# Bioconductor/SparseArray

Measured on AMD Instinct MI355X. Metric: GNZ/s, SVT crossprod(svt, dense) 1e6x1e4 @1% nnz, higher is better.
Workload: dtype f64

## Files before the change

include/svt_hip.h:

```cpp
#ifndef SVT_HIP_H
#define SVT_HIP_H

#include <stddef.h>
#include <stdint.h>

#ifdef __cplusplus
extern "C" {
#endif

#define SVT_UNSUPPORTED 1

#define SVT_LGLSXP 10
#define SVT_INTSXP 13
#define SVT_REALSXP 14

#define SVT_OP_ANYNA            1
#define SVT_OP_COUNTNAS         2
#define SVT_OP_ANY              3
#define SVT_OP_ALL              4
#define SVT_OP_MIN              5
#define SVT_OP_MAX              6
#define SVT_OP_RANGE            7
#define SVT_OP_SUM              8
#define SVT_OP_PROD             9
// ... 102 lines not shown
int svt_dev_crossprod_prepared(const svt_dev_csc *A, const void *ws, int K,
			       double *out, int64_t out_stride_c,
			       int64_t out_stride_k, void *stream);
int svt_dev_crossprod_csc_dense(const svt_dev_csc *A, const void *Y,
				int64_t ldY, int K, int tr_y, double *out,
				int64_t out_stride_c, int64_t out_stride_k,
				void *ws, size_t ws_bytes, void *stream);

typedef struct svt_dev_pbc svt_dev_pbc;
svt_dev_pbc *svt_dev_pbc_build(const svt_dev_csc *A, int CBW, int WPB, int logR);
void svt_dev_pbc_release(svt_dev_pbc *P);
void svt_dev_pbc_trim(void);
size_t svt_dev_pbc_bytes(const svt_dev_pbc *P);
size_t svt_dev_crossprod_pbc_ws_bytes(const svt_dev_pbc *P, int K);
int svt_dev_crossprod_pbc(const svt_dev_pbc *P, const svt_dev_csc *A,
			  const double *Y, int64_t ldY, int K, int tr_y,
			  double *out, int64_t out_stride_c,
			  int64_t out_stride_k, void *ws, size_t ws_bytes,
			  void *stream);

void svt_dev_pbc_set_spare_cus(int n);
int svt_dev_pbc_spare_cus(void);

void svt_dev_pbc_set_gather_pacing(int dsync, int spin);

void svt_dev_pbc_set_round_launches(int on);

int svt_dev_crossprod_pbc_from(const svt_dev_pbc *P, const svt_dev_csc *A,
			       const double *Y, int64_t ldY, int K, int tr_y,
			       double *out, int64_t out_stride_c,
			       int64_t out_stride_k, void *ws, size_t ws_bytes,
			       void *stream, int64_t first_col);

int svt_dev_crossprod_pbc_phase(const svt_dev_pbc *P, const svt_dev_csc *A,
				const double *Y, int64_t ldY, int K, int tr_y,
				double *out, int64_t out_stride_c,
				int64_t out_stride_k, void *ws, size_t ws_bytes,
				void *stream, int phase);

int svt_dev_colstats(const svt_dev_csc *A, int opcode, int na_rm,
		     double center, int64_t inner, void *out, int *warn_flag,
		     void *stream);

size_t svt_dev_colmedians_ws_bytes(int64_t nnz, int64_t ncol);
int svt_dev_colmedians(const svt_dev_csc *A, int na_rm, double *out, void *ws, size_t ws_bytes,
		       void *stream);
// ... 59 lines not shown
```

sparsearray_amd/_hip.py:

```python
from __future__ import annotations

import ctypes
import os

_HERE = os.path.dirname(os.path.abspath(__file__))
LIB_PATH = os.path.join(_HERE, "libsvt_hip_tuning.so" if os.environ.get("SVT_HIP_TUNING") == "1"
                        else "libsvt_hip.so")

EXPORTS = [
    "svt_init", "svt_last_error", "svt_device_arch", "svt_set_devices", "svt_get_devices", "svt_set_shard_min_nnz",
    "svt_crossprod2_SVT_mat", "svt_crossprod2_mat_SVT",
    "svt_crossprod2_SVT_SVT", "svt_crossprod1_SVT",
    "svt_matmul_SVT_mat", "svt_matmul_SVT_SVT", "svt_tcrossprod1_SVT", "svt_tcrossprod2_SVT_SVT",
    "svt_colMedians_SVT", "svt_rowMedians_SVT", "svt_dev_colmedians_ws_bytes", "svt_dev_colmedians",
    "svt_resident_set_limit", "svt_resident_clear", "svt_resident_stats", "svt_dev_pbc_bytes", "svt_dev_pbc_set_spare_cus", "svt_dev_pbc_spare_cus", "svt_dev_pbc_set_gather_pacing", "svt_dev_pbc_set_round_launches", "svt_dev_matmul_csc_csc_ws_bytes", "svt_dev_matmul_csc_csc", "svt_dev_rowsums_prepare", "svt_dev_rowsums_prepared", "svt_dev_rowsum_gid_bytes", "svt_dev_rowsum_prepare", "svt_dev_rowsum_prepared", "svt_dev_matmul_csc_csc_prepare", "svt_dev_matmul_csc_csc_prepared",
    "svt_dev_crossprod_csc_csc_ws_bytes", "svt_dev_crossprod_csc_csc", "svt_dev_crossprod_csc_csc_set_panel", "svt_sparse_crossprod_set_cost", "svt_dev_crossprod_csc_csc_dense_buffer",
    "svt_summarize_SVT", "svt_colStats_out_Rtype", "svt_colStats_SVT",
    "svt_rowStats_SVT", "svt_rowsum_SVT", "svt_colsum_SVT",
    "svt_rowsum_dgCMatrix", "svt_colsum_dgCMatrix",
    "svt_colMins_dgCMatrix", "svt_colMaxs_dgCMatrix", "svt_colRanges_dgCMatrix", "svt_colVars_dgCMatrix",
    "svt_upload", "svt_wrap_device_csc", "svt_release",
    "svt_dev_crossprod_ws_bytes", "svt_dev_crossprod_csc_dense",
    "svt_dev_dense_prepare", "svt_dev_crossprod_prepared",
    "svt_dev_pbc_build", "svt_dev_pbc_release", "svt_dev_pbc_trim",
    "svt_dev_crossprod_pbc_ws_bytes", "svt_dev_crossprod_pbc", "svt_dev_crossprod_pbc_phase", "svt_dev_crossprod_pbc_from",
    "svt_get_num_procs", "svt_get_max_threads", "svt_set_max_threads", "svt_dev_aperm_ws_bytes", "svt_dev_aperm_perm_ws_bytes", "svt_dev_aperm", "svt_dev_aperm_route_counts", "svt_aperm_SVT", "svt_transpose_2D_SVT", "svt_dev_transpose_ws_bytes", "svt_dev_transpose", "svt_dev_set_box_nnz", "svt_dev_boxed_calls", "svt_dev_colstats", "svt_dev_rowstats_ws_bytes", "svt_dev_rowsums", "svt_dev_rowsum",
]


class HipBackendError(RuntimeError):
    pass


_lib = None
_ready = False


def load_library() -> ctypes.CDLL:
# ... 59 lines not shown
```

sparsearray_amd/csrc/kernels_mult_pbc.hip:

```cpp
#include "svt_common.h"

#include <string.h>

#include <mutex>

#include "svt_scan.h"

typedef double d16 __attribute__((ext_vector_type(16)));
typedef double d8 __attribute__((ext_vector_type(8)));

struct svt_dev_pbc {
	int64_t nrow, ncol, nnz, nrec;
	int CBW, WPB, logR;
	int kind;
	int64_t ngroups, nblocks, npanels;
	uint4 *rec;
	int64_t *tile_ptr;
	int *col_has_na;
	int64_t max_leaf_nnz;
	mutable hipStream_t use_s[4];
	mutable int nuse;
	mutable bool use_overflow;
	int device;
};

#define PCH 256
__device__ inline int64_t pbc_stagger_batch(int stag_mode, int w, int64_t nb)
{
	const int g = w >> 2;
	switch (stag_mode) {
	case 0: return 0;
	case 1: return w & 1;
	case 2: return w & 3;
	case 3: return g & 1;
	case 4: return w & 7;
	case 5: return (w * nb) >> 4;
// ... 28 lines not shown
					  int64_t hi, int64_t key)
{
	while (lo < hi) {
		const int64_t mid = (lo + hi) >> 1;
		if ((int64_t) row[mid] < key) lo = mid + 1; else hi = mid;
	}
	return lo;
}

#define PBC_BATCH 4
#define PBC_SLACK 320
#define PBC_TP_PAD 8

__device__ inline void pbc1_store(uint4 *rec, int64_t ridx, uint32_t meta, double x)
{
	char *base = (char *) rec + (ridx >> 3) * 96;
	((uint32_t *) base)[ridx & 7] = meta;
	((double *) (base + 32))[ridx & 7] = x;
}

template <int MODE, int FMT>
__global__ void __launch_bounds__(64)
pbc_pass_kernel(const int64_t *__restrict__ col_ptr, const int32_t *__restrict__ row_idx,
		const double *__restrict__ val, int64_t ncol, int CBW, int logR,
		int64_t npanels, int64_t *__restrict__ counts_or_ptr,
		uint4 *__restrict__ rec, int *__restrict__ col_has_na, int stag_mode, int tile_flags)
{
	constexpr int BATCH = FMT == 1 ? 8 : PBC_BATCH;
	__shared__ int64_t fill[PCH];
	const int lane = threadIdx.x;
	const int64_t wv = blockIdx.x;
	const int64_t p0 = (int64_t) blockIdx.y * PCH;
	const int64_t p1 = p0 + PCH < npanels ? p0 + PCH : npanels;
#define TILE_OF(P) (wv * npanels + (P))
	for (int i = lane; i < PCH; i += 64)
		fill[i] = (MODE == 1 && p0 + i < npanels) ? counts_or_ptr[TILE_OF(p0 + i)] : 0;
	__syncthreads();
	const int64_t c0 = wv * CBW;
	const int64_t c1 = c0 + CBW < ncol ? c0 + CBW : ncol;
	for (int64_t c = c0; c < c1; c++) {
		const int64_t beg = col_ptr[c], end = col_ptr[c + 1];
		const int64_t lo = lower_bound_row(row_idx, beg, end, p0 << logR);
		const int64_t hi = lower_bound_row(row_idx, lo, end, p1 << logR);
		int saw_na = 0;
		for (int64_t k0 = lo; k0 < hi; k0 += 64) {
			const int64_t k = k0 + lane;
			const bool active = k < hi;
			const int32_t r = active ? row_idx[k] : 0;
			const int p = active ? (int) (((int64_t) r >> logR) - p0) : -1;
			const int prev_p = __shfl_up(p, 1, 64);
			const int next_p = __shfl_down(p, 1, 64);
			const bool is_first = active && (lane == 0 || p != prev_p);
			const bool is_last = active && (lane == 63 || p != next_p);
			const unsigned long long firsts = __ballot(is_first);
			const unsigned long long below = firsts & ((lane == 63) ? ~0ULL : ((2ULL << lane) - 1));
			const int seg_lane = 63 - __clzll(below | 1ULL);
			const int rank = lane - seg_lane;
			int64_t pos = 0;
			if (active) pos = fill[p] + rank;
			__syncthreads();
			if (MODE == 1 && active) {
				const double x = val[k];
// ... 37 lines not shown
				const int64_t nb = (stop - start) >> 3;
				int64_t bi = pbc_stagger_batch(stag_mode, w, nb);
				if (bi > nb - 1) bi = nb - 1;
				atomicOr((unsigned int *) ((char *) rec + ((start >> 3) + bi) * 96), 0x4000u);
			}
		}
	}
#undef TILE_OF
}

#define PBC_IMG_BYTES 24576
#define PBC_SC_KEEP 4

__device__ inline void pbc1_put(char *img, int64_t ridx, uint32_t meta, double x)
{
	char *b = img + (ridx >> 3) * 96;
	((uint32_t *) b)[ridx & 7] = meta;
	((double *) (b + 32))[ridx & 7] = x;
}

#define PBC_COUNT_MAXPANELS 36000
__global__ void __launch_bounds__(1024)
pbc_count_stream_kernel(const int64_t *__restrict__ col_ptr, const int32_t *__restrict__ row_idx, int64_t ncol,
			int CBW, int logR, int64_t npanels, int64_t *__restrict__ counts,
			int32_t *__restrict__ bounds, int64_t nchunks, int cshift)
{
	extern __shared__ uint32_t pbc_hist[];
	const int lane = threadIdx.x & 63, w = threadIdx.x >> 6;
	const int64_t g = blockIdx.x;
	for (int64_t p = threadIdx.x; p < npanels; p += 1024) pbc_hist[p] = 0;
	__syncthreads();
	const int64_t c0 = g * CBW, c1 = c0 + CBW < ncol ? c0 + CBW : ncol;
	for (int64_t c = c0 + w; c < c1; c += 16) {
		const int64_t beg = col_ptr[c], end = col_ptr[c + 1];
		int32_t *__restrict__ bc = bounds + c * (nchunks + 1);
		int64_t carry = -1;
		for (int64_t k0 = beg; k0 < end; k0 += 256) {
			int32_t r4[4];
#pragma unroll
			for (int u = 0; u < 4; u++) {
				const int64_t k = k0 + u * 64 + lane;
				r4[u] = k < end ? row_idx[k] : 0x7FFFFFFF;
			}
#pragma unroll
			for (int u = 0; u < 4; u++) {
				const int64_t kb = k0 + u * 64, k = kb + lane;
				if (kb >= end) break;
				const bool active = k < end;
				if (active) atomicAdd(&pbc_hist[r4[u] >> logR], 1u);
				const int64_t q = active ? (int64_t) (r4[u] >> cshift) : nchunks;
				int64_t pq = __shfl_up(q, 1, 64);
				if (lane == 0) pq = carry;
				carry = __shfl(q, 63, 64);
				if (k <= end)
					for (int64_t i = pq + 1; i <= q; i++) bc[i] = (int32_t) (k - beg);
// ... 5 lines not shown
		}
	}
	__syncthreads();
	for (int64_t p = threadIdx.x; p < npanels; p += 1024) {
		int64_t n = ((int64_t) pbc_hist[p] + 7) / 8 * 8;
		if (n == 0) n = 8;
		counts[g * npanels + p] = n;
	}
}

__global__ void pbc_bounds_kernel(const int64_t *__restrict__ col_ptr, const int32_t *__restrict__ row_idx,
				  int64_t ncol, int64_t nchunks, int64_t rows_per_chunk,
				  int32_t *__restrict__ bounds)
{
	const int64_t t = (int64_t) blockIdx.x * blockDim.x + threadIdx.x;
	if (t >= ncol * (nchunks + 1)) return;
	const int64_t c = t / (nchunks + 1), q = t - c * (nchunks + 1);
	const int64_t beg = col_ptr[c], end = col_ptr[c + 1];
	bounds[t] = (int32_t) (lower_bound_row(row_idx, beg, end, q * rows_per_chunk) - beg);
}

__global__ void __launch_bounds__(256)
pbc_scatter_lds_kernel(const int64_t *__restrict__ col_ptr, const int32_t *__restrict__ row_idx,
		       const double *__restrict__ val, int64_t ncol, int CBW, int logR, int64_t npanels,
		       const int64_t *__restrict__ tile_ptr, char *__restrict__ rec,
		       int *__restrict__ col_has_na, int stag_mode, int subp,
		       const int32_t *__restrict__ bounds, int64_t nchunks)
{
	extern __shared__ __attribute__((aligned(16))) char lds_raw[];
	char *img = lds_raw;
	int *s_cnt = (int *) (lds_raw + PBC_IMG_BYTES);
	int *s_first = s_cnt + subp * CBW;
	__shared__ int64_t s_lo[64];
	__shared__ int s_cum[65];
	__shared__ int s_tile0[257];
	const int tid = threadIdx.x;
	const int64_t g = blockIdx.x;
	const int64_t ps = (int64_t) blockIdx.y * subp;
	const int np = (int) (ps + subp <= npanels ? subp : npanels - ps);
	const int64_t c0 = g * CBW;
	const int nc = (int) (c0 + CBW <= ncol ? CBW : (c0 < ncol ? ncol - c0 : 0));
	const int64_t base = tile_ptr[g * npanels + ps];
	const int64_t nr = tile_ptr[g * npanels + ps + np] - base;
	const int64_t nbytes = (nr >> 3) * 96;
	const bool in_lds = nbytes <= PBC_IMG_BYTES;
	char *dst = in_lds ? img : rec + (base >> 3) * 96;
	if (tid < nc) {
		const int64_t c = c0 + tid;
		const int32_t *bc = bounds + c * (nchunks + 1) + blockIdx.y;
		s_lo[tid] = col_ptr[c] + bc[0];
		s_cum[tid + 1] = bc[1] - bc[0];
	}
	if (tid <= np) s_tile0[tid] = (int) (tile_ptr[g * npanels + ps + tid] - base);
	for (int i = tid; i < np * nc; i += 256) { s_cnt[i] = 0; s_first[i] = 0x7fffffff; }
	if (in_lds)
		for (int64_t i = tid; i < nbytes / 16; i += 256) ((uint4 *) img)[i] = make_uint4(0, 0, 0, 0);
	__syncthreads();
	if (tid == 0) {
		s_cum[0] = 0;
		for (int j = 0; j < nc; j++) s_cum[j + 1] += s_cum[j];
	}
	__syncthreads();
	const int total = s_cum[nc];
	int ka[PBC_SC_KEEP], kr[PBC_SC_KEEP];
// ... 200 lines not shown
	       (size_t) (h->ngroups * h->npanels + 1 + PBC_TP_PAD) * 8 + (size_t) h->ncol * 4;
}

void pbc_auto_layout(int64_t nrow, int64_t ncol, int64_t nnz, int *CBW, int *WPB, int *logR)
{
	*CBW = 40;
	const double per_tile = (double) nnz * 40.0 * 128.0 /
				((double) (nrow > 0 ? nrow : 1) * (double) (ncol > 0 ? ncol : 1));
	if (per_tile < 12.0 && nrow >= 4096) {
		*WPB = 4;
		*logR = (nrow >> 11) >= 64 ? 11 : (nrow >> 10) >= 64 ? 10 : 9;
	} else { *WPB = 16; *logR = 7; }
}

int pbc_kind(int64_t nrow, int CBW, int WPB, int logR)
{
	if (CBW < 1 || CBW > 40)
		return PBC_KIND_BAD;
	if (WPB == 16 && logR == 7)
		return nrow >= 256 && nrow < ((int64_t) 1 << 28) ? PBC_KIND_DMA : PBC_KIND_NONE;
	return WPB == 4 && logR >= 9 && logR <= 15 ? PBC_KIND_GATHER : PBC_KIND_BAD;
}

extern "C" svt_dev_pbc *svt_dev_pbc_build(const svt_dev_csc *A, int CBW, int WPB, int logR)
{
	if (A->Rtype != SVT_REALSXP) {
		svt_set_error("svt_dev_pbc_build: f64 operands only");
		return NULL;
	}
	if (CBW == 0 && WPB == 0 && logR == 0)
		pbc_auto_layout(A->nrow, A->ncol, A->nnz, &CBW, &WPB, &logR);
	const int kind = pbc_kind(A->nrow, CBW, WPB, logR);
	if (kind == PBC_KIND_BAD) {
		svt_set_error("svt_dev_pbc_build: no product kernel reads the layout (CBW %d, WPB %d, logR %d): "
			      "(CBW <= 40, 16, 7) for the LDS-DMA kernel or (CBW <= 40, 4, 9 .. 15) for the gather kernels",
			      CBW, WPB, logR);
		return NULL;
	}
	svt_dev_pbc *h = (svt_dev_pbc *) calloc(1, sizeof(*h));
	h->nrow = A->nrow; h->ncol = A->ncol; h->nnz = A->nnz;
	h->CBW = CBW; h->WPB = WPB; h->logR = logR;
	h->kind = kind;
	const bool dma = kind == PBC_KIND_DMA;
	const int64_t CB = (int64_t) CBW * WPB;
	h->nblocks = (A->ncol + CB - 1) / CB;
	h->ngroups = h->nblocks * WPB;
	h->npanels = (A->nrow + (1LL << logR) - 1) >> logR;
	if (h->npanels < 1) h->npanels = 1;
	const int64_t ntiles = h->ngroups * h->npanels;
	if (ntiles + 1 + PBC_TP_PAD >= (int64_t) 2147483647) {
		svt_set_error("svt_dev_pbc_build: too many tiles (%lld) for the panel-blocked layout",
			      (long long) ntiles);
		free(h);
		return NULL;
	}
	void *tmp = NULL;
	int32_t *bounds = NULL;
	size_t tmp_bytes = 0;
	bool ok = pbc_alloc((void **) &h->tile_ptr, (size_t) (ntiles + 1 + PBC_TP_PAD) * 8) == hipSuccess &&
		  pbc_alloc((void **) &h->col_has_na, (size_t) (A->ncol > 0 ? A->ncol : 1) * 4) == hipSuccess;
	if (ok) ok = hipMemsetAsync(h->tile_ptr, 0, (size_t) (ntiles + 1 + PBC_TP_PAD) * 8, 0) == hipSuccess &&
		     hipMemsetAsync(h->col_has_na, 0, (size_t) (A->ncol > 0 ? A->ncol : 1) * 4, 0) == hipSuccess;
	int subp = 16;
	while (subp < 128 && (double) A->nnz * subp < 8.0 * (double) A->ncol * (double) h->npanels)
		subp *= 2;
	const int64_t nchunks = (h->npanels + subp - 1) / subp;
	const int64_t nb_entries = A->ncol * (nchunks + 1);
	bool bounds_done = false;
	if (ok && kind != PBC_KIND_NONE && A->ncol > 0 && A->nnz > 0) {
		const int BATCH = dma ? 8 : PBC_BATCH;
		const size_t rbytes = dma ? 12 : 16;
		const int64_t nrec_max = A->nnz + ntiles * (int64_t) BATCH;
		dim3 grid((unsigned) h->ngroups, (unsigned) ((h->npanels + PCH - 1) / PCH));
		if (dma && h->npanels <= PBC_COUNT_MAXPANELS) {
			ok = pbc_alloc((void **) &bounds, (size_t) nb_entries * 4) == hipSuccess;
			if (ok) {
				int sl = 0;
				while ((1 << sl) < subp) sl++;
				const size_t lds = (size_t) h->npanels * 4;
				(void) hipFuncSetAttribute((const void *) pbc_count_stream_kernel,
							   hipFuncAttributeMaxDynamicSharedMemorySize, (int) lds);
				hipLaunchKernelGGL(pbc_count_stream_kernel, dim3((unsigned) h->ngroups), dim3(1024), lds, 0,
						   A->col_ptr, A->row_idx, A->ncol, CBW, logR, h->npanels, h->tile_ptr,
						   bounds, nchunks, logR + sl);
				bounds_done = true;
			}
		} else if (dma)
			hipLaunchKernelGGL((pbc_pass_kernel<0, 1>), grid, dim3(64), 0, 0, A->col_ptr, A->row_idx,
					   (const double *) A->val, A->ncol, CBW, logR, h->npanels,
					   h->tile_ptr, (uint4 *) NULL, h->col_has_na, g_pbc_stagger, 0);
		else
			hipLaunchKernelGGL((pbc_pass_kernel<0, 0>), grid, dim3(64), 0, 0, A->col_ptr, A->row_idx,
					   (const double *) A->val, A->ncol, CBW, logR, h->npanels,
					   h->tile_ptr, (uint4 *) NULL, h->col_has_na, g_pbc_stagger, 1);
		tmp_bytes = exclusive_scan_ws_bytes(ntiles + 1);
		ok = pbc_alloc(&tmp, tmp_bytes) == hipSuccess &&
		     launch_exclusive_scan_i64(h->tile_ptr, ntiles + 1, tmp, 0) == 0;
		if (ok) ok = pbc_alloc((void **) &h->rec, (size_t) nrec_max * rbytes + PBC_SLACK * 16) == hipSuccess;
		if (ok) {
			if (dma) {
				if (!bounds_done) ok = pbc_alloc((void **) &bounds, (size_t) nb_entries * 4) == hipSuccess;
				if (ok) {
					if (!bounds_done)
						hipLaunchKernelGGL(pbc_bounds_kernel, dim3((unsigned) ((nb_entries + 255) / 256)), dim3(256), 0, 0,
								   A->col_ptr, A->row_idx, A->ncol, nchunks, (int64_t) subp << logR, bounds);
					const size_t lds = PBC_IMG_BYTES + (size_t) 2 * subp * CBW * 4;
					(void) hipFuncSetAttribute((const void *) pbc_scatter_lds_kernel,
								   hipFuncAttributeMaxDynamicSharedMemorySize, (int) lds);
					dim3 sgrid((unsigned) h->ngroups, (unsigned) nchunks);
					hipLaunchKernelGGL(pbc_scatter_lds_kernel, sgrid, dim3(256), lds, 0, A->col_ptr, A->row_idx,
							   (const double *) A->val, A->ncol, CBW, logR, h->npanels,
							   h->tile_ptr, (char *) h->rec, h->col_has_na, g_pbc_stagger, subp,
							   bounds, nchunks);
				}
			} else {
				hipLaunchKernelGGL((pbc_pass_kernel<1, 0>), grid, dim3(64), 0, 0, A->col_ptr,
						   A->row_idx, (const double *) A->val, A->ncol, CBW, logR,
						   h->npanels, h->tile_ptr, h->rec, h->col_has_na, g_pbc_stagger, 1);
			}
		}
		long long hmeta[3] = {0, 0, 0};
		bool too_big = false;
		if (ok) {
			long long *meta = (long long *) tmp;
			ok = hipMemsetAsync(meta, 0, 24, 0) == hipSuccess;
			if (ok) {
				hipLaunchKernelGGL(pbc_max_leaf_kernel, dim3((unsigned) ((A->ncol + 255) / 256 < 512 ? (A->ncol + 255) / 256 : 512)), dim3(256), 0, 0,
						   A->col_ptr, A->ncol, (unsigned long long *) (meta + 1));
				hipLaunchKernelGGL(pbc_group_limit_kernel, dim3((unsigned) ((h->ngroups + 255) / 256)),
						   dim3(256), 0, 0, h->tile_ptr, h->npanels, h->ngroups, (int *) (meta + 2));
				hipLaunchKernelGGL(pbc_build_finish_kernel, dim3(1), dim3(256), 0, 0, h->tile_ptr, ntiles,
						   (char *) h->rec, (int) rbytes, meta);
				ok = hipMemcpy(hmeta, meta, 24, hipMemcpyDeviceToHost) == hipSuccess;
			}
			h->nrec = hmeta[0];
			h->max_leaf_nnz = hmeta[1];
			too_big = hmeta[2] != 0;
		}
		if (ok && too_big) {
			svt_set_error("svt_dev_pbc_build: a column group too large for 32-bit record offsets");
// ... 349 lines not shown
		if constexpr (NV > 2) {
#pragma unroll
			for (int jj = 0; jj < 8; jj++)
				if (32 + jj < CBW && c0 + 32 + jj < ncol) {
					dlo[32 + jj] = acc8[jj];
					dhi[32 + jj] = acch8[jj];
				}
		}
	}
	if (lane == 0)
		__hip_atomic_store(pg_mine, PBGX_DONE, __ATOMIC_RELAXED, __HIP_MEMORY_SCOPE_AGENT);
}

#include "pbc_dma_asm.inc"
typedef uint32_t u32x16 __attribute__((ext_vector_type(16)));
typedef uint32_t u32x4 __attribute__((ext_vector_type(4)));
typedef uint32_t u32x8 __attribute__((ext_vector_type(8)));
#define PBC_DMA_CLOBBERS "memory", "scc", "vcc", "s28", "s29", "s30", "s31", "s32", "s33", "s34", "s35", "s36", "s37", "s38", "s39", "s40", "s41", "s42", "s43", "s44", "s45", "s46", "s47", "s48", "s49", "s50", "s51", "s52", "s53", "s54", "s55", "s56", "s57", "s58", "s59", "s60", "s61", "s62", "s63", "s64", "s65", "s66", "s67", "s68", "s69", "s70", "s71", "s72", "s73", "s74", "s75", "s76", "s77", "s78", "s79", "s80", "s81", "s82", "s83", "s84", "s85", "s86", "s87", "s88", "s89", "s90", "s91", "s92", "s93", "s94", "s95", "s96", "s97", "s98", "s99"

template <int NV, int PROF>
__global__ void __launch_bounds__(1024)
crossprod_pbc_dma_kernel(const uint4 *__restrict__ rec, const int64_t *__restrict__ tile_ptr,
			 int64_t npanels, const double *__restrict__ Y, int64_t ldY, int64_t nrow,
			 int K, int64_t ncol, int CBW, int nfull, int nblocks, int block0,
			 int64_t panels_per_split, double *__restrict__ part, int64_t Kp,
			 PbcFlags fl, int rt_lines, int rt_ahead, int stag_mode, int64_t part_ld, int64_t part_c0)
{
	extern __shared__ double ylds[];
	const int tid = threadIdx.x;
	const int w = __builtin_amdgcn_readfirstlane(tid >> 6);
	const int kt = (int) (Kp / 64);
	const int L = blockIdx.x;
#ifdef SVT_TUNING
	unsigned long long t_entry = 0, t_loop = 0, t_epi = 0;
	if (PROF) t_entry = __builtin_readcyclecounter();
#endif
	int bl, kh, split;
	if (nfull < 0) {
		const int V = (L & 7) * (-nfull) + (L >> 3), u = V / nblocks;
		bl = V % nblocks; kh = u % kt; split = u / kt;
	} else if (L < nfull * kt * nblocks) {
		const int xcd = L & 7, j = L >> 3, u = j / nblocks;
		bl = j % nblocks; kh = u % kt; split = (u / kt) * 8 + xcd;
	} else {
		const int Lr = L - nfull * kt * nblocks, u = Lr / nblocks;
		bl = Lr % nblocks; kh = u % kt; split = nfull + u / kt;
	}
// ... 111 lines not shown
			     : : PBC_DMA_CLOBBERS);
	} else if constexpr (NV == 2) {
		asm volatile(PBC_DMA_ASM_TEXT
			     : PBC_ACC0(acc[0]), PBC_ACC1(acc[NV > 1 ? 1 : 0]), PBC_DMA_STATE
			     : : PBC_DMA_CLOBBERS);
	} else {
		asm volatile(PBC_DMA_ASM_TEXT
			     : PBC_ACC0(acc[0]), PBC_ACC1(acc[NV > 1 ? 1 : 0]),
			       PBC_ACC2(acc8), PBC_DMA_STATE
			     : : PBC_DMA_CLOBBERS);
	}
#undef PBC_ACC0
#undef PBC_ACC1
#undef PBC_ACC2
#undef PBC_DMA_STATE
	if (PB[6] != 0 && (tid & 63) == 0) {
		*fl.y_nonfinite = 1;
		fl.y_nonfinite[PBC_SUBFLAG0 + (split * kt + kh) % PBC_NSUBFLAG] = 1;
	}
#ifdef SVT_TUNING
	if (PROF) t_epi = __builtin_readcyclecounter();
#endif
	const int lane2 = (int) __builtin_amdgcn_mbcnt_hi(~0u, __builtin_amdgcn_mbcnt_lo(~0u, 0u));
	const int CWG = 16 * CBW, LS = CWG + 2;
	const int64_t cwg0 = (int64_t) b * CWG;
	const int nvalid = (int) (ncol - cwg0 < CWG ? ncol - cwg0 : CWG);
	__syncthreads();
#pragma unroll 1
	for (int q = 0; q < 4; q++) {
		if ((lane2 >> 4) == q) {
			double *row = ylds + (lane2 & 15) * LS + w * CBW;
#pragma unroll
			for (int ii = 0; ii < (NV > 2 ? 2 : NV); ii++)
#pragma unroll
				for (int jj = 0; jj < 16; jj++)
					if (ii * 16 + jj < CBW) row[ii * 16 + jj] = acc[ii][jj];
			if constexpr (NV > 2) {
#pragma unroll
				for (int jj = 0; jj < 8; jj++)
					if (32 + jj < CBW) row[32 + jj] = acc8[jj];
			}
		}
		__syncthreads();
		{
			double *__restrict__ dstrow = part + ((int64_t) split * Kp + k0 + q * 16 + w) * part_ld + (cwg0 - part_c0);
			const double *__restrict__ src = ylds + w * LS;
			if ((((uintptr_t) dstrow) & 15) == 0) {
				for (int cc = lane2 * 2; cc < nvalid; cc += 128) {
					if (cc + 1 < nvalid) *(double2 *) (dstrow + cc) = *(const double2 *) (src + cc);
					else dstrow[cc] = src[cc];
				}
			} else {
				for (int cc = lane2; cc < nvalid; cc += 64) dstrow[cc] = src[cc];
			}
		}
		__syncthreads();
	}
#ifdef SVT_TUNING
	if (PROF && tid == 0 && (blockIdx.x == 0 || blockIdx.x == gridDim.x - 1 || blockIdx.x == gridDim.x / 2)) {
		const unsigned long long t_end = __builtin_readcyclecounter();
		printf("wg %d: prologue %llu, panel loop %llu, epilogue %llu cycles\n", (int) blockIdx.x,
		       t_loop - t_entry, t_epi - t_loop, t_end - t_epi);
	}
#endif
}


__global__ void __launch_bounds__(256)
pbc_transpose_dense_kernel(const double *__restrict__ Yin, int64_t ldY, int64_t nrow, int K,
			   double *__restrict__ Yc)
{
	__shared__ double tile[64][65];
	const int tx = threadIdx.x & 63, ty = threadIdx.x >> 6;
	const int k0 = blockIdx.y * 64;
	for (int64_t r0 = (int64_t) blockIdx.x * 64; r0 < nrow; r0 += (int64_t) gridDim.x * 64) {
		if (r0 != (int64_t) blockIdx.x * 64) __syncthreads();
// ... 408 lines not shown
	const size_t lds = (size_t) 2 * PBC_DMA_BUF;
	const int kt = (int) (Kp / 64);
	const double tile_bytes = P->ngroups * P->npanels > 0 ?
		(double) P->nrec * 12.0 / (double) (P->ngroups * P->npanels) : 0.0;
	int rt_lines = (int) (tile_bytes * 1.5 / 128.0) + 2;
	if (rt_lines > 31) rt_lines = 31;
	int rt_ahead = ((int) (g_pbc_ahead10 * 0.1 * tile_bytes) + 127) / 128 * 128;
	if (rt_ahead + rt_lines * 128 > 4608) rt_ahead = 4608 - rt_lines * 128;
	if (rt_ahead < 0) rt_ahead = 0;
#ifdef SVT_TUNING
	auto kern = g_pbc_debug != 3 ? crossprod_pbc_dma_kernel<NV, 0> :
		    NV <= 2 ? crossprod_pbc_dma_kernel<(NV <= 2 ? NV : 2), 1> : crossprod_pbc_dma_kernel<NV, 2>;
#else
	auto kern = crossprod_pbc_dma_kernel<NV, 0>;
#endif
	(void) hipFuncSetAttribute((const void *) kern, hipFuncAttributeMaxDynamicSharedMemorySize, (int) lds);
	int nb = (int) P->nblocks - block0;
	if (nb_launch > 0 && nb_launch < nb) nb = nb_launch;
	const bool sparing = pbc_sparing(P, K) && part_c0 == 0 && part_ld == P->ncol;
	const int per_xcd = (256 - g_pbc_spare_cus) / 8;
	const int nfull = sparing ? -per_xcd : nsplit & ~7;
	const int64_t nwg = sparing ? (int64_t) 8 * per_xcd : (int64_t) nsplit * kt * nb;
	hipLaunchKernelGGL(kern, dim3((unsigned) nwg), dim3(1024), lds, s,
			   P->rec, P->tile_ptr, P->npanels, Y, ldY, P->nrow, K, P->ncol, P->CBW, nfull,
			   nb, block0, pps, part, Kp, fl, rt_lines, rt_ahead, g_pbc_stagger, part_ld, part_c0);
}

__global__ void __launch_bounds__(256)
pbc_tail_reduce_kernel(const double *__restrict__ tail, int nsplit, int64_t Kp, int K, int64_t ld, int64_t ncols,
		       double *__restrict__ out, int64_t out_ld, int64_t c0)
{
	const int64_t c = ((int64_t) blockIdx.x * blockDim.x + threadIdx.x) * 2;
	const int k = blockIdx.y;
	if (c >= ncols || k >= K)
		return;
	if (c + 1 < ncols && ((out_ld | c0) & 1) == 0 && (((uintptr_t) out) & 15) == 0 && (((uintptr_t) tail) & 15) == 0) {
		double2 a = make_double2(0.0, 0.0);
		for (int t = 0; t < nsplit; t++) {
			const double2 v = *(const double2 *) (tail + ((int64_t) t * Kp + k) * ld + c);
			a.x += v.x; a.y += v.y;
		}
		*(double2 *) (out + (int64_t) k * out_ld + c0 + c) = a;
		return;
	}
	for (int64_t cc = c; cc < c + 2 && cc < ncols; cc++) {
		double a = 0.0;
		for (int t = 0; t < nsplit; t++) a += tail[((int64_t) t * Kp + k) * ld + cc];
		out[(int64_t) k * out_ld + c0 + cc] = a;
	}
}

__global__ void __launch_bounds__(256)
pbc_clear_kernel(uint32_t *__restrict__ a, int na, uint32_t *__restrict__ b, int nb, uint32_t *__restrict__ c, int nc)
{
	for (int i = threadIdx.x; i < na; i += blockDim.x) a[i] = 0u;
	if (b != NULL)
		for (int i = threadIdx.x; i < nb; i += blockDim.x) b[i] = 0u;
	if (c != NULL)
		for (int i = threadIdx.x; i < nc; i += blockDim.x) c[i] = 0u;
// ... 16 lines not shown
	const int rc = pbc_phase_impl(P, A, Y, ldY, K, tr_y, out, out_stride_c, out_stride_k, ws, ws_bytes, stream,
				      phase, first_col);
	pbc_note_use(P, (hipStream_t) stream);
	return rc;
}
static int pbc_phase_impl(const svt_dev_pbc *P, const svt_dev_csc *A,
			  const double *Y, int64_t ldY, int K, int tr_y,
			  double *out, int64_t out_stride_c,
			  int64_t out_stride_k, void *ws, size_t ws_bytes,
			  void *stream, int phase, int64_t first_col)
{
	hipStream_t s = (hipStream_t) stream;
	if (P->ncol <= 0 || K <= 0)
		return 0;
	if (ws_bytes < svt_dev_crossprod_pbc_ws_bytes(P, K))
		return svt_set_error("svt_dev_crossprod_pbc: workspace too small");
	const int64_t Kp = ((int64_t) K + 63) / 64 * 64;
	int64_t pps = 1;
	const int kind = P->rec != NULL ? P->kind : PBC_KIND_NONE;
	const bool dma = kind == PBC_KIND_DMA, gath = kind == PBC_KIND_GATHER;
	const bool via_copy = tr_y && dma;
	int block0 = 0;
	if (dma && first_col > 0) {
		block0 = (int) (first_col / ((int64_t) 16 * P->CBW));
		if (block0 > P->nblocks - 1) block0 = (int) P->nblocks - 1;
	}
	const int64_t c_begin = (int64_t) block0 * 16 * P->CBW;
	const int nsplit = gath ? pick_nsplit_gather(P, K, &pps) : dma ? pick_nsplit(P, K, &pps) : 0;
	PbcFlags fl;
	fl.y_nonfinite = (int *) ws;
	double *part = (double *) ((char *) ws + PBC_FLAG_BYTES);
	void *gen_ws = (char *) part + (size_t) nsplit * Kp * P->ncol * 8;
	const size_t gen_bytes = crossprod_ws_bytes(pbc_padded_rows(P), P->ncol, K);
	DirtyWs dw = dirty_ws_of(ws, (char *) gen_ws + gen_bytes, P->ncol, Kp);
	const double *Yc = via_copy ? (const double *) gen_ws : Y;
	const int64_t ldc = via_copy ? P->nrow : ldY;
	const bool direct = nsplit == 1 && Kp == K && out_stride_c == 1 && out_stride_k == P->ncol;
	if (direct) part = out;
	if (phase == 1) {
		{
			const bool paced = gath && pbgx_ok(P, K);
			hipLaunchKernelGGL(pbc_clear_kernel, dim3(1), dim3(256), 0, s,
					   (uint32_t *) ws, 64, (uint32_t *) dw.col_nf, (int) (Kp * 2),
					   paced ? (uint32_t *) ((char *) ws + PBC_PROG_OFFSET) : (uint32_t *) NULL,
					   8 * PBGX_PROG_ENTRIES);
		}
		if (kind == PBC_KIND_NONE) {
			HIP_TRY(hipMemsetAsync(ws, 1, 12, s));
			return 0;
		}
// ... 43 lines not shown
			return 0;
		}
		if (via_copy && P->nrow > 0) {
			const int64_t ntile = (P->nrow + 63) / 64;
			dim3 tg((unsigned) (ntile < 8192 ? ntile : 8192), (unsigned) (Kp / 64));
			hipLaunchKernelGGL(pbc_transpose_dense_kernel, tg, dim3(256), 0, s, Y, ldY, P->nrow, K,
					   (double *) gen_ws);
		}
		const int kt_ = (int) (Kp / 64);
		int per_launch = 0;
		if (nsplit == 1 && !pbc_sparing(P, K) && g_pbc_rounds != 0 &&
		    (int64_t) (P->nblocks - block0) * kt_ >= 2 * pbc_cus())
			per_launch = pbc_cus() / kt_ > 0 ? pbc_cus() / kt_ : 1;
		int tail_blocks = 0, ts = 1;
		int64_t tpps = pps;
		if (per_launch > 0 && direct && g_pbc_rounds == 1) {
			const int rem = (int) ((P->nblocks - block0) % per_launch);
			if (rem > 0 && rem * kt_ * 2 <= pbc_cus()) {
				ts = pbc_cus() / (rem * kt_);
				if (ts > 8) ts = 8;
				while (ts > 1 && P->npanels / ts < 8) ts--;
				tpps = (P->npanels + ts - 1) / ts;
				ts = (int) ((P->npanels + tpps - 1) / tpps);
				const int64_t tcols = (int64_t) rem * 16 * P->CBW;
				if (ts > 1 && (int64_t) ts * tcols <= P->ncol)
					tail_blocks = rem;
			}
		}
		const int last_full = (int) P->nblocks - tail_blocks;
		for (int b0 = block0; b0 < last_full; b0 += per_launch > 0 ? per_launch : (int) P->nblocks) {
			const int nbl = per_launch > 0 ? (b0 + per_launch <= last_full ? per_launch : last_full - b0)
						       : tail_blocks > 0 ? last_full - b0 : 0;
			if (nv == 1) launch_dma<1>(P, Yc, ldc, K, nsplit, pps, part, Kp, fl, s, b0, nbl);
			else if (nv == 2) launch_dma<2>(P, Yc, ldc, K, nsplit, pps, part, Kp, fl, s, b0, nbl);
			else launch_dma<3>(P, Yc, ldc, K, nsplit, pps, part, Kp, fl, s, b0, nbl);
		}
		if (tail_blocks > 0) {
			double *tail = (double *) ((char *) ws + PBC_FLAG_BYTES);
			const int64_t c0 = (int64_t) last_full * 16 * P->CBW;
			const int64_t tld = (int64_t) tail_blocks * 16 * P->CBW;
			const int64_t tcols = P->ncol - c0;
			if (nv == 1) launch_dma<1>(P, Yc, ldc, K, ts, tpps, tail, Kp, fl, s, last_full, tail_blocks, tld, c0);
			else if (nv == 2) launch_dma<2>(P, Yc, ldc, K, ts, tpps, tail, Kp, fl, s, last_full, tail_blocks, tld, c0);
			else launch_dma<3>(P, Yc, ldc, K, ts, tpps, tail, Kp, fl, s, last_full, tail_blocks, tld, c0);
			dim3 tg((unsigned) ((tcols + 511) / 512), (unsigned) K);
			hipLaunchKernelGGL(pbc_tail_reduce_kernel, tg, dim3(256), 0, s, tail, ts, Kp, K, tld, tcols,
					   out, P->ncol, c0);
		}
		HIP_TRY(hipGetLastError());
		return 0;
	}
	if (kind == PBC_KIND_NONE) {
		CrossprodArgs a;
		memset(&a, 0, sizeof(a));
		a.col_ptr = A->col_ptr; a.row_idx = A->row_idx; a.val = A->val; a.Rtype = SVT_REALSXP;
		a.nrow = A->nrow; a.ncol = A->ncol; a.Y = Y; a.ldY = ldY; a.K = K; a.tr_y = tr_y;
		a.out = out; a.out_stride_c = out_stride_c; a.out_stride_k = out_stride_k;
		a.ws = gen_ws; a.ws_bytes = gen_bytes;
		return launch_crossprod_general_if(a, fl.y_nonfinite, false, s);
	}
	const double *Yd = gath ? (const double *) gen_ws : Yc;
	const int64_t yrs = gath ? Kp : 1, ycs = gath ? 1 : ldc;
	DirtyScanArgs ds;
// ... 55 lines not shown
```

sparsearray_amd/device.py:

```python
from __future__ import annotations

import ctypes
from ctypes import c_double, c_int, c_int64, c_size_t, c_void_p

import numpy as np
import torch

from . import _hip
from .api import OPCODES, SparseArrayError, SparseArrayUnsupported
from .svt import INTSXP, LGLSXP, REALSXP

_protos_done = False


def _lib():
    global _protos_done
    lib = _hip.init()
    if not _protos_done:
        lib.svt_wrap_device_csc.restype = c_void_p
        lib.svt_wrap_device_csc.argtypes = [c_int, c_int64, c_int64, c_int64,
                                            c_void_p, c_void_p, c_void_p]
        lib.svt_release.argtypes = [c_void_p]
        lib.svt_release.restype = None
        lib.svt_dev_crossprod_ws_bytes.restype = c_size_t
        lib.svt_dev_crossprod_ws_bytes.argtypes = [c_int64, c_int64, c_int]
        lib.svt_dev_dense_prepare.argtypes = [c_void_p, c_int64, c_int64, c_int, c_int,
                                              c_int, c_void_p, c_size_t, c_void_p]
        lib.svt_dev_crossprod_prepared.argtypes = [c_void_p, c_void_p, c_int, c_void_p,
                                                   c_int64, c_int64, c_void_p]
        lib.svt_dev_crossprod_csc_dense.argtypes = [c_void_p, c_void_p, c_int64, c_int,
                                                    c_int, c_void_p, c_int64, c_int64,
                                                    c_void_p, c_size_t, c_void_p]
        lib.svt_dev_pbc_build.restype = c_void_p
        lib.svt_dev_pbc_build.argtypes = [c_void_p, c_int, c_int, c_int]
        lib.svt_dev_pbc_release.argtypes = [c_void_p]
        lib.svt_dev_pbc_release.restype = None
        lib.svt_dev_pbc_set_spare_cus.argtypes = [c_int]
        lib.svt_dev_pbc_set_spare_cus.restype = None
        lib.svt_dev_pbc_spare_cus.restype = c_int
        lib.svt_dev_pbc_set_gather_pacing.argtypes = [c_int, c_int]
        lib.svt_dev_pbc_set_gather_pacing.restype = None
        lib.svt_dev_crossprod_pbc_ws_bytes.restype = c_size_t
        lib.svt_dev_crossprod_pbc_ws_bytes.argtypes = [c_void_p, c_int]
        lib.svt_dev_crossprod_pbc.argtypes = [c_void_p, c_void_p, c_void_p, c_int64, c_int,
                                              c_int, c_void_p, c_int64, c_int64, c_void_p,
                                              c_size_t, c_void_p]
        lib.svt_dev_crossprod_pbc_phase.argtypes = [c_void_p, c_void_p, c_void_p, c_int64, c_int,
                                                    c_int, c_void_p, c_int64, c_int64, c_void_p,
                                                    c_size_t, c_void_p, c_int]
        lib.svt_dev_colstats.argtypes = [c_void_p, c_int, c_int, c_double, c_int64,
                                         c_void_p, c_void_p, c_void_p]
        lib.svt_dev_matmul_csc_csc_ws_bytes.restype = c_size_t
        lib.svt_dev_matmul_csc_csc_ws_bytes.argtypes = [c_void_p]
        lib.svt_dev_matmul_csc_csc.argtypes = [c_void_p, c_void_p, c_void_p, c_int64, c_void_p, c_size_t,
                                               c_void_p, c_void_p]
        lib.svt_dev_matmul_csc_csc_prepare.argtypes = [c_void_p, c_void_p, c_size_t, c_void_p]
        lib.svt_dev_matmul_csc_csc_prepared.argtypes = [c_void_p, c_void_p, c_void_p, c_int64, c_void_p, c_size_t,
                                                        c_void_p, c_void_p]
        lib.svt_dev_crossprod_csc_csc_ws_bytes.restype = c_size_t
        lib.svt_dev_crossprod_csc_csc_ws_bytes.argtypes = [c_void_p]
        lib.svt_dev_crossprod_csc_csc.argtypes = [c_void_p, c_void_p, c_int, c_void_p, c_int64, c_void_p, c_size_t,
                                                  c_void_p, c_void_p]
# ... 121 lines not shown
            stride_k = self.A.ncol
        self.prepare(Y, ldY, tr_y)
        self.multiply(out, stride_c, stride_k)


class PbcPlan:

    def __init__(self, A: DeviceCSC, K: int, CBW: int = 40, WPB: int = 16, logR: int = 7):
        assert A.Rtype == REALSXP
        self.A, self.K = A, int(K)
        self._p = _lib().svt_dev_pbc_build(A.handle, CBW, WPB, logR)
        if not self._p:
            raise SparseArrayError(_lib().svt_last_error().decode())
        n = _lib().svt_dev_crossprod_pbc_ws_bytes(self._p, self.K)
        self.ws = torch.empty(n, dtype=torch.uint8, device=A.val.device)

    def run(self, Y, ldY, out, stride_c=1, stride_k=None, tr_y=False):
        if stride_k is None:
            stride_k = self.A.ncol
        _check(_lib().svt_dev_crossprod_pbc(self._p, self.A.handle, Y.data_ptr(), ldY, self.K,
                                            int(tr_y), out.data_ptr(), stride_c, stride_k,
                                            self.ws.data_ptr(), self.ws.numel(), _stream()))

    def run_phase(self, phase, Y, ldY, out, stride_c=1, stride_k=None, tr_y=False):
        if stride_k is None:
            stride_k = self.A.ncol
        _check(_lib().svt_dev_crossprod_pbc_phase(self._p, self.A.handle, Y.data_ptr(), ldY,
                                                  self.K, int(tr_y), out.data_ptr(), stride_c,
                                                  stride_k, self.ws.data_ptr(), self.ws.numel(),
                                                  _stream(), phase))

    def __del__(self):
        try:
            if getattr(self, "_p", None):
                _lib().svt_dev_pbc_release(self._p)
                self._p = None
        except Exception:
            pass


def aperm_route_counts(reset=False) -> dict:
    names = ("t_bucketed", "t_key_sort", "leaf_preserving", "first_two_axes_swapped", "slab", "via_intermediate_3d",
             "general_composed", "key_sort_32", "key_sort_64", "slab_refused_at_run_time")
    buf = (c_int64 * 10)()
    _lib().svt_dev_aperm_route_counts.argtypes = [c_void_p, c_int]
    _lib().svt_dev_aperm_route_counts.restype = None
    _lib().svt_dev_aperm_route_counts(buf, int(bool(reset)))
    return dict(zip(names, (int(x) for x in buf)))


def set_box_nnz(n: int = 0) -> None:
    _lib().svt_dev_set_box_nnz(int(n))


def boxed_calls(reset=False) -> int:
    return int(_lib().svt_dev_boxed_calls(int(bool(reset))))


def trim_layout_pool() -> None:
    _lib().svt_dev_pbc_trim.restype = None
    _lib().svt_dev_pbc_trim()


def set_spare_cus(n: int) -> None:
    _lib().svt_dev_pbc_set_spare_cus(int(n))


def spare_cus() -> int:
    return int(_lib().svt_dev_pbc_spare_cus())


def set_gather_pacing(dsync: int = 1, spin: int = 256) -> None:
    _lib().svt_dev_pbc_set_gather_pacing(int(dsync), int(spin))


def set_round_launches(on=True) -> None:
    _lib().svt_dev_pbc_set_round_launches.restype = None
    _lib().svt_dev_pbc_set_round_launches(int(on))


def crossprod_csc_dense(A: DeviceCSC, Y: torch.Tensor) -> torch.Tensor:
    K, nrow = Y.shape
    assert nrow == A.nrow and Y.is_contiguous()
    out = torch.zeros((K, A.ncol), dtype=torch.float64, device=Y.device)
    CrossprodPlan(A, K).run(Y, nrow, out)
    return out


def colstats(A: DeviceCSC, op: str, na_rm=False, center=float("nan"), inner=1):
    oc = OPCODES[op]
    rt = _lib().svt_colStats_out_Rtype(oc, A.Rtype)
    nseg = A.ncol // inner
# ... 135 lines not shown
```

Baseline: 57.13.

## Balance PBC column groups evenly across all groups instead of fixed CBW width

Replaces the fixed CBW-column-per-group partition with an even split of ncol across ngroups (base plus remainder) in the DMA path, threading a PbcCols layout through the build, count, scatter and crossprod kernels. The goal is to remove the ragged last block, where a few groups held leftover columns and the others idled. The epilogue also aligns LDS staging to the destination's 16-byte alignment so the double2 store path is always used. Column-to-block mapping, the tail-block logic and the first_col lookup are all rewritten, so there is some risk of off-by-one errors at group boundaries.

```diff
diff --git a/include/svt_hip.h b/include/svt_hip.h
--- a/include/svt_hip.h
+++ b/include/svt_hip.h
@@ -148,6 +148,9 @@
 void svt_dev_pbc_set_spare_cus(int n);
 int svt_dev_pbc_spare_cus(void);
 
+void svt_dev_pbc_set_even_groups(int on);
+int svt_dev_pbc_even_groups(void);
+
 void svt_dev_pbc_set_gather_pacing(int dsync, int spin);
 
 void svt_dev_pbc_set_round_launches(int on);
diff --git a/sparsearray_amd/_hip.py b/sparsearray_amd/_hip.py
--- a/sparsearray_amd/_hip.py
+++ b/sparsearray_amd/_hip.py
@@ -13,7 +13,7 @@
     "svt_crossprod2_SVT_SVT", "svt_crossprod1_SVT",
     "svt_matmul_SVT_mat", "svt_matmul_SVT_SVT", "svt_tcrossprod1_SVT", "svt_tcrossprod2_SVT_SVT",
     "svt_colMedians_SVT", "svt_rowMedians_SVT", "svt_dev_colmedians_ws_bytes", "svt_dev_colmedians",
-    "svt_resident_set_limit", "svt_resident_clear", "svt_resident_stats", "svt_dev_pbc_bytes", "svt_dev_pbc_set_spare_cus", "svt_dev_pbc_spare_cus", "svt_dev_pbc_set_gather_pacing", "svt_dev_pbc_set_round_launches", "svt_dev_matmul_csc_csc_ws_bytes", "svt_dev_matmul_csc_csc", "svt_dev_rowsums_prepare", "svt_dev_rowsums_prepared", "svt_dev_rowsum_gid_bytes", "svt_dev_rowsum_prepare", "svt_dev_rowsum_prepared", "svt_dev_matmul_csc_csc_prepare", "svt_dev_matmul_csc_csc_prepared",
+    "svt_resident_set_limit", "svt_resident_clear", "svt_resident_stats", "svt_dev_pbc_bytes", "svt_dev_pbc_set_spare_cus", "svt_dev_pbc_spare_cus", "svt_dev_pbc_set_even_groups", "svt_dev_pbc_even_groups", "svt_dev_pbc_set_gather_pacing", "svt_dev_pbc_set_round_launches", "svt_dev_matmul_csc_csc_ws_bytes", "svt_dev_matmul_csc_csc", "svt_dev_rowsums_prepare", "svt_dev_rowsums_prepared", "svt_dev_rowsum_gid_bytes", "svt_dev_rowsum_prepare", "svt_dev_rowsum_prepared", "svt_dev_matmul_csc_csc_prepare", "svt_dev_matmul_csc_csc_prepared",
     "svt_dev_crossprod_csc_csc_ws_bytes", "svt_dev_crossprod_csc_csc", "svt_dev_crossprod_csc_csc_set_panel", "svt_sparse_crossprod_set_cost", "svt_dev_crossprod_csc_csc_dense_buffer",
     "svt_summarize_SVT", "svt_colStats_out_Rtype", "svt_colStats_SVT",
     "svt_rowStats_SVT", "svt_rowsum_SVT", "svt_colsum_SVT",
diff --git a/sparsearray_amd/csrc/kernels_mult_pbc.hip b/sparsearray_amd/csrc/kernels_mult_pbc.hip
--- a/sparsearray_amd/csrc/kernels_mult_pbc.hip
+++ b/sparsearray_amd/csrc/kernels_mult_pbc.hip
@@ -8,10 +8,30 @@
 
 typedef double d16 __attribute__((ext_vector_type(16)));
 typedef double d8 __attribute__((ext_vector_type(8)));
+
+struct PbcCols {
+	int64_t base, rem;
+};
+__host__ __device__ inline int64_t pbc_group_first(const PbcCols L, int64_t g)
+{
+	return g * L.base + (g < L.rem ? g : L.rem);
+}
+__host__ __device__ inline int64_t pbc_group_of(const PbcCols L, int64_t c)
+{
+	const int64_t wide = L.rem * (L.base + 1);
+	return c < wide ? c / (L.base + 1) : L.base > 0 ? L.rem + (c - wide) / L.base : L.rem;
+}
+__host__ __device__ inline int64_t pbc_group_cols(const PbcCols L, int64_t g, int64_t ncol, int64_t *c0)
+{
+	const int64_t a = pbc_group_first(L, g), b = pbc_group_first(L, g + 1);
+	*c0 = a < ncol ? a : ncol;
+	return b < ncol ? b : ncol;
+}
 
 struct svt_dev_pbc {
 	int64_t nrow, ncol, nnz, nrec;
 	int CBW, WPB, logR;
+	PbcCols cols;
 	int kind;
 	int64_t ngroups, nblocks, npanels;
 	uint4 *rec;
@@ -86,7 +106,7 @@
 template <int MODE, int FMT>
 __global__ void __launch_bounds__(64)
 pbc_pass_kernel(const int64_t *__restrict__ col_ptr, const int32_t *__restrict__ row_idx,
-		const double *__restrict__ val, int64_t ncol, int CBW, int logR,
+		const double *__restrict__ val, int64_t ncol, PbcCols cols, int logR,
 		int64_t npanels, int64_t *__restrict__ counts_or_ptr,
 		uint4 *__restrict__ rec, int *__restrict__ col_has_na, int stag_mode, int tile_flags)
 {
@@ -100,8 +120,8 @@
 	for (int i = lane; i < PCH; i += 64)
 		fill[i] = (MODE == 1 && p0 + i < npanels) ? counts_or_ptr[TILE_OF(p0 + i)] : 0;
 	__syncthreads();
-	const int64_t c0 = wv * CBW;
-	const int64_t c1 = c0 + CBW < ncol ? c0 + CBW : ncol;
+	int64_t c0;
+	const int64_t c1 = pbc_group_cols(cols, wv, ncol, &c0);
 	for (int64_t c = c0; c < c1; c++) {
 		const int64_t beg = col_ptr[c], end = col_ptr[c + 1];
 		const int64_t lo = lower_bound_row(row_idx, beg, end, p0 << logR);
@@ -185,7 +205,7 @@
 #define PBC_COUNT_MAXPANELS 36000
 __global__ void __launch_bounds__(1024)
 pbc_count_stream_kernel(const int64_t *__restrict__ col_ptr, const int32_t *__restrict__ row_idx, int64_t ncol,
-			int CBW, int logR, int64_t npanels, int64_t *__restrict__ counts,
+			PbcCols cols, int logR, int64_t npanels, int64_t *__restrict__ counts,
 			int32_t *__restrict__ bounds, int64_t nchunks, int cshift)
 {
 	extern __shared__ uint32_t pbc_hist[];
@@ -193,7 +213,8 @@
 	const int64_t g = blockIdx.x;
 	for (int64_t p = threadIdx.x; p < npanels; p += 1024) pbc_hist[p] = 0;
 	__syncthreads();
-	const int64_t c0 = g * CBW, c1 = c0 + CBW < ncol ? c0 + CBW : ncol;
+	int64_t c0;
+	const int64_t c1 = pbc_group_cols(cols, g, ncol, &c0);
 	for (int64_t c = c0 + w; c < c1; c += 16) {
 		const int64_t beg = col_ptr[c], end = col_ptr[c + 1];
 		int32_t *__restrict__ bc = bounds + c * (nchunks + 1);
@@ -245,7 +266,7 @@
 
 __global__ void __launch_bounds__(256)
 pbc_scatter_lds_kernel(const int64_t *__restrict__ col_ptr, const int32_t *__restrict__ row_idx,
-		       const double *__restrict__ val, int64_t ncol, int CBW, int logR, int64_t npanels,
+		       const double *__restrict__ val, int64_t ncol, PbcCols cols, int CBW, int logR, int64_t npanels,
 		       const int64_t *__restrict__ tile_ptr, char *__restrict__ rec,
 		       int *__restrict__ col_has_na, int stag_mode, int subp,
 		       const int32_t *__restrict__ bounds, int64_t nchunks)
@@ -261,8 +282,8 @@
 	const int64_t g = blockIdx.x;
 	const int64_t ps = (int64_t) blockIdx.y * subp;
 	const int np = (int) (ps + subp <= npanels ? subp : npanels - ps);
-	const int64_t c0 = g * CBW;
-	const int nc = (int) (c0 + CBW <= ncol ? CBW : (c0 < ncol ? ncol - c0 : 0));
+	int64_t c0;
+	const int nc = (int) (pbc_group_cols(cols, g, ncol, &c0) - c0);
 	const int64_t base = tile_ptr[g * npanels + ps];
 	const int64_t nr = tile_ptr[g * npanels + ps + np] - base;
 	const int64_t nbytes = (nr >> 3) * 96;
@@ -509,6 +530,10 @@
 	return WPB == 4 && logR >= 9 && logR <= 15 ? PBC_KIND_GATHER : PBC_KIND_BAD;
 }
 
+static int g_pbc_even_groups = 1;
+extern "C" void svt_dev_pbc_set_even_groups(int on) { g_pbc_even_groups = on ? 1 : 0; }
+extern "C" int svt_dev_pbc_even_groups(void) { return g_pbc_even_groups; }
+
 extern "C" svt_dev_pbc *svt_dev_pbc_build(const svt_dev_csc *A, int CBW, int WPB, int logR)
 {
 	if (A->Rtype != SVT_REALSXP) {
@@ -532,6 +557,12 @@
 	const int64_t CB = (int64_t) CBW * WPB;
 	h->nblocks = (A->ncol + CB - 1) / CB;
 	h->ngroups = h->nblocks * WPB;
+	h->cols.base = CBW; h->cols.rem = 0;
+	if (dma && g_pbc_even_groups && h->ngroups > 0) {
+		h->cols.base = A->ncol / h->ngroups;
+		h->cols.rem = A->ncol % h->ngroups;
+	}
+	const PbcCols cols = h->cols;
 	h->npanels = (A->nrow + (1LL << logR) - 1) >> logR;
 	if (h->npanels < 1) h->npanels = 1;
 	const int64_t ntiles = h->ngroups * h->npanels;
@@ -568,17 +599,17 @@
 				(void) hipFuncSetAttribute((const void *) pbc_count_stream_kernel,
 							   hipFuncAttributeMaxDynamicSharedMemorySize, (int) lds);
 				hipLaunchKernelGGL(pbc_count_stream_kernel, dim3((unsigned) h->ngroups), dim3(1024), lds, 0,
-						   A->col_ptr, A->row_idx, A->ncol, CBW, logR, h->npanels, h->tile_ptr,
+						   A->col_ptr, A->row_idx, A->ncol, cols, logR, h->npanels, h->tile_ptr,
 						   bounds, nchunks, logR + sl);
 				bounds_done = true;
 			}
 		} else if (dma)
 			hipLaunchKernelGGL((pbc_pass_kernel<0, 1>), grid, dim3(64), 0, 0, A->col_ptr, A->row_idx,
-					   (const double *) A->val, A->ncol, CBW, logR, h->npanels,
+					   (const double *) A->val, A->ncol, cols, logR, h->npanels,
 					   h->tile_ptr, (uint4 *) NULL, h->col_has_na, g_pbc_stagger, 0);
 		else
 			hipLaunchKernelGGL((pbc_pass_kernel<0, 0>), grid, dim3(64), 0, 0, A->col_ptr, A->row_idx,
-					   (const double *) A->val, A->ncol, CBW, logR, h->npanels,
+					   (const double *) A->val, A->ncol, cols, logR, h->npanels,
 					   h->tile_ptr, (uint4 *) NULL, h->col_has_na, g_pbc_stagger, 1);
 		tmp_bytes = exclusive_scan_ws_bytes(ntiles + 1);
 		ok = pbc_alloc(&tmp, tmp_bytes) == hipSuccess &&
@@ -596,13 +627,13 @@
 								   hipFuncAttributeMaxDynamicSharedMemorySize, (int) lds);
 					dim3 sgrid((unsigned) h->ngroups, (unsigned) nchunks);
 					hipLaunchKernelGGL(pbc_scatter_lds_kernel, sgrid, dim3(256), lds, 0, A->col_ptr, A->row_idx,
-							   (const double *) A->val, A->ncol, CBW, logR, h->npanels,
+							   (const double *) A->val, A->ncol, cols, CBW, logR, h->npanels,
 							   h->tile_ptr, (char *) h->rec, h->col_has_na, g_pbc_stagger, subp,
 							   bounds, nchunks);
 				}
 			} else {
 				hipLaunchKernelGGL((pbc_pass_kernel<1, 0>), grid, dim3(64), 0, 0, A->col_ptr,
-						   A->row_idx, (const double *) A->val, A->ncol, CBW, logR,
+						   A->row_idx, (const double *) A->val, A->ncol, cols, logR,
 						   h->npanels, h->tile_ptr, h->rec, h->col_has_na, g_pbc_stagger, 1);
 			}
 		}
@@ -998,7 +1029,7 @@
 __global__ void __launch_bounds__(1024)
 crossprod_pbc_dma_kernel(const uint4 *__restrict__ rec, const int64_t *__restrict__ tile_ptr,
 			 int64_t npanels, const double *__restrict__ Y, int64_t ldY, int64_t nrow,
-			 int K, int64_t ncol, int CBW, int nfull, int nblocks, int block0,
+			 int K, int64_t ncol, PbcCols cols, int CBW, int nfull, int nblocks, int block0,
 			 int64_t panels_per_split, double *__restrict__ part, int64_t Kp,
 			 PbcFlags fl, int rt_lines, int rt_ahead, int stag_mode, int64_t part_ld, int64_t part_c0)
 {
@@ -1156,36 +1187,39 @@
 	if (PROF) t_epi = __builtin_readcyclecounter();
 #endif
 	const int lane2 = (int) __builtin_amdgcn_mbcnt_hi(~0u, __builtin_amdgcn_mbcnt_lo(~0u, 0u));
-	const int CWG = 16 * CBW, LS = CWG + 2;
-	const int64_t cwg0 = (int64_t) b * CWG;
-	const int nvalid = (int) (ncol - cwg0 < CWG ? ncol - cwg0 : CWG);
+	const int LS = 16 * CBW + 2;
+	int64_t cwg0, clast0;
+	(void) pbc_group_cols(cols, (int64_t) b * 16, ncol, &cwg0);
+	const int nvalid = (int) (pbc_group_cols(cols, (int64_t) b * 16 + 15, ncol, &clast0) - cwg0);
+	const int wc0 = (int) (pbc_group_first(cols, wv) - pbc_group_first(cols, (int64_t) b * 16));
+	const int gw = (int) (pbc_group_first(cols, wv + 1) - pbc_group_first(cols, wv));
+	auto part_row = [&](int r) { return part + ((int64_t) split * Kp + k0 + r) * part_ld + (cwg0 - part_c0); };
 	__syncthreads();
 #pragma unroll 1
 	for (int q = 0; q < 4; q++) {
 		if ((lane2 >> 4) == q) {
-			double *row = ylds + (lane2 & 15) * LS + w * CBW;
+			const int mis = (int) (((uintptr_t) part_row(q * 16 + (lane2 & 15)) >> 3) & 1);
+			double *row = ylds + (lane2 & 15) * LS + mis + wc0;
 #pragma unroll
 			for (int ii = 0; ii < (NV > 2 ? 2 : NV); ii++)
 #pragma unroll
 				for (int jj = 0; jj < 16; jj++)
-					if (ii * 16 + jj < CBW) row[ii * 16 + jj] = acc[ii][jj];
+					if (ii * 16 + jj < gw) row[ii * 16 + jj] = acc[ii][jj];
 			if constexpr (NV > 2) {
 #pragma unroll
 				for (int jj = 0; jj < 8; jj++)
-					if (32 + jj < CBW) row[32 + jj] = acc8[jj];
+					if (32 + jj < gw) row[32 + jj] = acc8[jj];
 			}
 		}
 		__syncthreads();
 		{
-			double *__restrict__ dstrow = part + ((int64_t) split * Kp + k0 + q * 16 + w) * part_ld + (cwg0 - part_c0);
-			const double *__restrict__ src = ylds + w * LS;
-			if ((((uintptr_t) dstrow) & 15) == 0) {
-				for (int cc = lane2 * 2; cc < nvalid; cc += 128) {
-					if (cc + 1 < nvalid) *(double2 *) (dstrow + cc) = *(const double2 *) (src + cc);
-					else dstrow[cc] = src[cc];
-				}
-			} else {
-				for (int cc = lane2; cc < nvalid; cc += 64) dstrow[cc] = src[cc];
+			double *__restrict__ dstrow = part_row(q * 16 + w);
+			const int mis = (int) (((uintptr_t) dstrow >> 3) & 1);
+			const double *__restrict__ src = ylds + w * LS + mis;
+			if (mis && lane2 == 0 && nvalid > 0) dstrow[0] = src[0];
+			for (int cc = mis + lane2 * 2; cc < nvalid; cc += 128) {
+				if (cc + 1 < nvalid) *(double2 *) (dstrow + cc) = *(const double2 *) (src + cc);
+				else dstrow[cc] = src[cc];
 			}
 		}
 		__syncthreads();
@@ -1640,7 +1674,7 @@
 	const int nfull = sparing ? -per_xcd : nsplit & ~7;
 	const int64_t nwg = sparing ? (int64_t) 8 * per_xcd : (int64_t) nsplit * kt * nb;
 	hipLaunchKernelGGL(kern, dim3((unsigned) nwg), dim3(1024), lds, s,
-			   P->rec, P->tile_ptr, P->npanels, Y, ldY, P->nrow, K, P->ncol, P->CBW, nfull,
+			   P->rec, P->tile_ptr, P->npanels, Y, ldY, P->nrow, K, P->ncol, P->cols, P->CBW, nfull,
 			   nb, block0, pps, part, Kp, fl, rt_lines, rt_ahead, g_pbc_stagger, part_ld, part_c0);
 }
 
@@ -1652,7 +1686,7 @@
 	const int k = blockIdx.y;
 	if (c >= ncols || k >= K)
 		return;
-	if (c + 1 < ncols && ((out_ld | c0) & 1) == 0 && (((uintptr_t) out) & 15) == 0 && (((uintptr_t) tail) & 15) == 0) {
+	if (c + 1 < ncols && ((out_ld | c0 | ld) & 1) == 0 && (((uintptr_t) out) & 15) == 0 && (((uintptr_t) tail) & 15) == 0) {
 		double2 a = make_double2(0.0, 0.0);
 		for (int t = 0; t < nsplit; t++) {
 			const double2 v = *(const double2 *) (tail + ((int64_t) t * Kp + k) * ld + c);
@@ -1715,10 +1749,10 @@
 	const bool via_copy = tr_y && dma;
 	int block0 = 0;
 	if (dma && first_col > 0) {
-		block0 = (int) (first_col / ((int64_t) 16 * P->CBW));
+		block0 = first_col < P->ncol ? (int) (pbc_group_of(P->cols, first_col) / 16) : (int) P->nblocks - 1;
 		if (block0 > P->nblocks - 1) block0 = (int) P->nblocks - 1;
 	}
-	const int64_t c_begin = (int64_t) block0 * 16 * P->CBW;
+	const int64_t c_begin = pbc_group_first(P->cols, (int64_t) block0 * 16);
 	const int nsplit = gath ? pick_nsplit_gather(P, K, &pps) : dma ? pick_nsplit(P, K, &pps) : 0;
 	PbcFlags fl;
 	fl.y_nonfinite = (int *) ws;
@@ -1808,7 +1842,8 @@
 				while (ts > 1 && P->npanels / ts < 8) ts--;
 				tpps = (P->npanels + ts - 1) / ts;
 				ts = (int) ((P->npanels + tpps - 1) / tpps);
-				const int64_t tcols = (int64_t) rem * 16 * P->CBW;
+				const int64_t tcols = pbc_group_first(P->cols, P->ngroups) -
+						      pbc_group_first(P->cols, (P->nblocks - rem) * 16);
 				if (ts > 1 && (int64_t) ts * tcols <= P->ncol)
 					tail_blocks = rem;
 			}
@@ -1823,8 +1858,8 @@
 		}
 		if (tail_blocks > 0) {
 			double *tail = (double *) ((char *) ws + PBC_FLAG_BYTES);
-			const int64_t c0 = (int64_t) last_full * 16 * P->CBW;
-			const int64_t tld = (int64_t) tail_blocks * 16 * P->CBW;
+			const int64_t c0 = pbc_group_first(P->cols, (int64_t) last_full * 16);
+			const int64_t tld = pbc_group_first(P->cols, P->ngroups) - c0;
 			const int64_t tcols = P->ncol - c0;
 			if (nv == 1) launch_dma<1>(P, Yc, ldc, K, ts, tpps, tail, Kp, fl, s, last_full, tail_blocks, tld, c0);
 			else if (nv == 2) launch_dma<2>(P, Yc, ldc, K, ts, tpps, tail, Kp, fl, s, last_full, tail_blocks, tld, c0);
diff --git a/sparsearray_amd/device.py b/sparsearray_amd/device.py
--- a/sparsearray_amd/device.py
+++ b/sparsearray_amd/device.py
@@ -38,6 +38,12 @@
         lib.svt_dev_pbc_set_spare_cus.argtypes = [c_int]
         lib.svt_dev_pbc_set_spare_cus.restype = None
         lib.svt_dev_pbc_spare_cus.restype = c_int
+        lib.svt_dev_pbc_set_even_groups.argtypes = [c_int]
+        lib.svt_dev_pbc_set_even_groups.restype = None
+        lib.svt_dev_pbc_even_groups.restype = c_int
+        lib.svt_dev_crossprod_pbc_from.argtypes = [c_void_p, c_void_p, c_void_p, c_int64, c_int,
+                                                   c_int, c_void_p, c_int64, c_int64, c_void_p,
+                                                   c_size_t, c_void_p, c_int64]
         lib.svt_dev_pbc_set_gather_pacing.argtypes = [c_int, c_int]
         lib.svt_dev_pbc_set_gather_pacing.restype = None
         lib.svt_dev_crossprod_pbc_ws_bytes.restype = c_size_t
@@ -205,6 +211,14 @@
                                             int(tr_y), out.data_ptr(), stride_c, stride_k,
                                             self.ws.data_ptr(), self.ws.numel(), _stream()))
 
+    def run_from(self, first_col, Y, ldY, out, stride_c=1, stride_k=None, tr_y=False):
+        if stride_k is None:
+            stride_k = self.A.ncol
+        _check(_lib().svt_dev_crossprod_pbc_from(self._p, self.A.handle, Y.data_ptr(), ldY, self.K,
+                                                 int(tr_y), out.data_ptr(), stride_c, stride_k,
+                                                 self.ws.data_ptr(), self.ws.numel(), _stream(),
+                                                 int(first_col)))
+
     def run_phase(self, phase, Y, ldY, out, stride_c=1, stride_k=None, tr_y=False):
         if stride_k is None:
             stride_k = self.A.ncol
@@ -251,6 +265,14 @@
 
 def spare_cus() -> int:
     return int(_lib().svt_dev_pbc_spare_cus())
+
+
+def set_even_groups(on=True) -> None:
+    _lib().svt_dev_pbc_set_even_groups(int(bool(on)))
+
+
+def even_groups() -> bool:
+    return bool(_lib().svt_dev_pbc_even_groups())
 
 
 def set_gather_pacing(dsync: int = 1, spin: int = 256) -> None:
```

New measurement: 56.59. No clear change (-1.0%).
